# tobifinn/torch-assimilate

Hardware: AMD Instinct MI355X
Metric: local analyses/sec (LETKF, 40-member) (higher is better)
Workload: dtype f32

## Files before the change

torch-assimilate_amd/csrc/letkf_tile2_kernel.h:

```cpp
#pragma once
#include <type_traits>
#include "mia_common.h"
#include <hip/hip_ext.h>
#include "mia_kernels.h"
#include "mia_options.h"
#include "mia_tiles.h"
#ifdef MIA_TILE_STAMPS
namespace mia { constexpr int kT2StampN = 20, kT2StampTiles = 8192; static __device__ long long g_tile2_stamps[kT2StampTiles * kT2StampN]; }
#define MIA_TL_STAMP(i) do { if (lane == 0 && tile < mia::kT2StampTiles) mia::g_tile2_stamps[tile * mia::kT2StampN + 12 + (i)] = (long long)__builtin_amdgcn_s_memtime(); } while (0)
#endif
#include "mia_tile_localize.h"

namespace mia {

#ifdef MIA_TILE_STAMPS
#define T2_STAMP(i) do { if (lane == 0 && bid < kT2StampTiles) g_tile2_stamps[bid * kT2StampN + (i)] = (long long)__builtin_amdgcn_s_memtime(); } while (0)
#define T2_STAMP_HWID() do { if (lane == 0 && bid < kT2StampTiles) g_tile2_stamps[bid * kT2StampN + 9] = \
    (long long)(unsigned)__builtin_amdgcn_s_getreg((31 << 11) | 4) | ((long long)(unsigned)__builtin_amdgcn_s_getreg((31 << 11) | 20) << 32); } while (0)
#define T2_STAMP_REAL(i) do { if (lane == 0 && bid < kT2StampTiles) g_tile2_stamps[bid * kT2StampN + (i)] = (long long)__builtin_amdgcn_s_memrealtime(); } while (0)
#else
#define T2_STAMP(i) do { } while (0)
#define T2_STAMP_HWID() do { } while (0)
#define T2_STAMP_REAL(i) do { } while (0)
#endif

#ifndef MIA_TILE2_WAVES_UT2
#define MIA_TILE2_WAVES_UT2 4
#endif

template <int UT, int KT, bool MROWS, int LOC>
__device__ __forceinline__ void tile2_body(Tile2Params P, const Tile2Loc* loc, const int64_t bid) {
  constexpr int UMAX = 16 * UT, NB = (KT + 1) / 2, NKB = (UT + 1) / 2;
  extern __shared__ __attribute__((aligned(16))) unsigned char smem[];
  int lane = threadIdx.x, lr = lane & 15, h = lane >> 4;
  const int k = P.k, nc8 = P.nc8;
  const unsigned IMG = (unsigned)(UT * nc8) * 512u;
  unsigned char* zline = smem + IMG;
  int* ukey = reinterpret_cast<int*>(smem + IMG + 512);
  float* wdl = reinterpret_cast<float*>(ukey + UMAX);
  float* El = wdl + UMAX;

  const int64_t ntile = (P.ng + 15) >> 4;
  if (bid >= ntile) return;
  if (P.clr_counts) {
    const int ncl = *P.clr_n;
    for (int64_t i = bid * 64 + lane; i < ncl; i += ntile * 64) P.clr_counts[i] = 0;
    if (bid == 0 && lane == 0) {
      const unsigned e = *P.clr_err;
      if (e) { atomicOr(P.err_out, (int)(e << 3)); *P.clr_err = 0u; }
    }
  }
  const int64_t q8 = ntile >> 3, r8 = ntile & 7, xcd = bid & 7;
  const int64_t tile = (xcd < r8 ? xcd * (q8 + 1) : r8 * (q8 + 1) + (xcd - r8) * q8) + (bid >> 3);
  const int64_t p0 = tile << 4;
  const int npts = P.ng - p0 < 16 ? (int)(P.ng - p0) : 16;
  int64_t oc0 = P.o0 + p0;
  if (P.seg_len > 0) {
    const unsigned sgi = (unsigned)p0 / (unsigned)P.seg_len;
    oc0 = p0 - (int64_t)sgi * P.seg_len;
    P.Xa += (int64_t)sgi * P.seg_stride;
  }
  const unsigned ldxb = (unsigned)P.ldx * 4u, ldob = (unsigned)P.ldo * 4u;
  int lrc = lr < npts ? lr : npts - 1;
  bool colok = lr < npts;

#ifdef MIA_EXPERIMENTS
  const int prio_mode = (P.stagger >> 8) & 0xff, exp_trim = P.stagger >> 16;
  P.stagger &= 0xff;
  if (prio_mode == 1) __builtin_amdgcn_s_setprio(3);
  if (prio_mode >= 3) {
    const int wid = (int)(__builtin_amdgcn_s_getreg((4 << 11) | 4) & 0xf);
    const bool fast = prio_mode == 3 ? (wid & 1) : (prio_mode == 4 ? wid < 2 : (prio_mode == 5 ? wid == 0 : (wid % 3) == 0));
    if (fast) __builtin_amdgcn_s_setprio(3);
  }
  if (P.stagger > 0) {
    const int slot = (int)(__builtin_amdgcn_s_getreg((4 << 11) | 4) & 0xf);
    for (int i = 0; i < slot * P.stagger; ++i) __builtin_amdgcn_s_sleep(1);
  }
#endif
  T2_STAMP(0);
  T2_STAMP_HWID();
  T2_STAMP_REAL(10);
  int hdU = 0;
  int myidx[(UMAX + 63) / 64];
  f4w dreg[UT];
  if constexpr (LOC == 0) {
    const int4 hd = P.thdr[tile];
    hdU = hd.x;
#pragma unroll
    for (int r = 0; r < (UMAX + 63) / 64; ++r) {
      const int s = lane + 64 * r;
      myidx[r] = s < UMAX ? t2_ld<int32_t>(P.tidx + tile * UMAX, (unsigned)s * 4u) : -1;
    }
#pragma unroll
    for (int t = 0; t < UT; ++t) dreg[t] = t2_ld<f4w>(P.tD + (tile * UT + t) * 64, (unsigned)lane * 16u);
  } else {
    const TileLocOut lo = tile_localize<true, (LOC > 3 ? LOC - 4 : LOC), MIA_TAPER_GC, (LOC > 3)>(loc->scan, P.g0, P.ng, UT, tile, smem, lane);
    const TileLocLds LL(smem);
    hdU = lo.overflow ? -1 : lo.U;
    int mu[(UMAX + 63) / 64], du[UT][4];
#pragma unroll
    for (int r = 0; r < (UMAX + 63) / 64; ++r) {
      const int s = lane + 64 * r;
      mu[r] = LL.uinv[s < UMAX ? s : 0];
      mu[r] = (s < UMAX && !lo.overflow && mu[r] >= 0) ? mu[r] : kTlUmax;
    }
#pragma unroll
    for (int t = 0; t < UT; ++t)
#pragma unroll
      for (int qq = 0; qq < 4; ++qq) {
        du[t][qq] = LL.uinv[16 * t + 4 * h + qq];
        du[t][qq] = (!lo.overflow && du[t][qq] >= 0) ? du[t][qq] * 16 + lr : LL.zrow_off + lr;
      }
#pragma unroll
    for (int r = 0; r < (UMAX + 63) / 64; ++r) myidx[r] = LL.ukey[mu[r]];
#pragma unroll
    for (int t = 0; t < UT; ++t) {
      f4w v;
#pragma unroll
      for (int qq = 0; qq < 4; ++qq) v[qq] = LL.Wt[du[t][qq]];
      dreg[t] = v;
    }
    if (lane == 0) {
      if (lo.longest > loc->longest_bound) atomicMax(&loc->stats[0], lo.longest);
      else if ((tile & 63) == 0 && lo.longest > __hip_atomic_load(&loc->stats[0], __ATOMIC_RELAXED, __HIP_MEMORY_SCOPE_AGENT))
        atomicMax(&loc->stats[0], lo.longest);
      if (tile == 0) atomicOr(&loc->stats[3], kStepSampledLongest);
      if (lo.overflow) atomicAdd(&loc->stats[1], 1);
      if (lo.box_overflow) atomicOr(&loc->stats[1], MIA_TILE_BOX_OVERFLOW);
    }
    MIA_T2_SYNC();
  }
  int sg = 2 * (h & 1) + (h >> 1);
  auto load_xs = [&](int mi, float (&xr)[NB][8]) {
    const float* xbase = P.X + (int64_t)mi * k * P.ldx + P.g0 + p0;
#pragma unroll
    for (int b = 0; b < NB; ++b) {
      const int m0 = 8 * (4 * b + sg);
      if (b < NB - 1 || (k & 7) == 0) {
        const unsigned vo = (unsigned)(m0 < k ? m0 : 0) * ldxb + (unsigned)lrc * 4u;
#pragma unroll
        for (int i = 0; i < 8; ++i) xr[b][i] = t2_ld<float>(xbase, vo + (unsigned)i * ldxb);
      } else {
#pragma unroll
        for (int i = 0; i < 8; ++i) {
          const int mem = m0 + i;
          xr[b][i] = t2_ld<float>(xbase, (unsigned)(mem < k ? mem : k - 1) * ldxb + (unsigned)lrc * 4u);
        }
      }
    }
  };
  float xsb[NB][8];
  load_xs(0, xsb);
#pragma unroll
  for (int r = 0; r < (UMAX + 63) / 64; ++r) {
    const int s = lane + 64 * r;
    if (s < UMAX) ukey[s] = myidx[r];
  }
  for (int i = lane; i < 32; i += 64) reinterpret_cast<f4w*>(zline)[i] = f4w{0.f, 0.f, 0.f, 0.f};
  MIA_T2_SYNC();
  const int U = __builtin_amdgcn_readfirstlane(hdU);
  if (U < 0) {
    if (colok && h == 0) P.flags[p0 + lr] = MIA_FLAG_OVERFLOW;
    const float nanv = __builtin_nanf("");
    if (colok)
      for (int it = h; it < P.m * k; it += 4) P.Xa[(int64_t)it * P.ldo + oc0 + lr] = nanv;
    return;
  }
  T2_STAMP(1);
  {
    const int g = lane >> 4, hl = g & 1, gh = g >> 1;
    unsigned roff[UT][2];
#pragma unroll
    for (int t = 0; t < UT; ++t)
#pragma unroll
      for (int par = 0; par < 2; ++par) {
        const int idx = ukey[16 * t + ((lr - 8 * par) & 15)];
        roff[t][par] = (unsigned)(idx < 0 ? (int)P.zero_rec : idx) * (unsigned)P.rb + 16u * (unsigned)hl;
      }
    auto gather = [&](auto nc8c) {
      constexpr int NC8 = decltype(nc8c)::value;
      constexpr int NL = (UT * NC8 + 1) / 2;
#pragma unroll
      for (int u = 0; u < NL; ++u) {
        const int lA = 2 * u, lB = 2 * u + 1;
        const int tA = lA / NC8, cA = lA % NC8, tB = (lB / NC8) < UT ? lB / NC8 : UT - 1, cB = lB % NC8;
        const unsigned offA = roff[tA][cA & 1] + 32u * (unsigned)cA, offB = roff[tB][cB & 1] + 32u * (unsigned)cB;
        const unsigned off = gh ? offB : offA;
        const bool valid = 2 * u + gh < UT * NC8;
        if (valid)
          __builtin_amdgcn_global_load_lds(reinterpret_cast<const unsigned*>(P.rec + off),
                                           (__attribute__((address_space(3))) void*)(smem + u * 1024), 16, 0, 0);
      }
    };
    if (nc8 == 2 * KT - 1) gather(std::integral_constant<int, 2 * KT - 1>{});
    else gather(std::integral_constant<int, 2 * KT>{});
  }
  f2w tails[(UMAX + 63) / 64];
#pragma unroll
  for (int r = 0; r < (UMAX + 63) / 64; ++r) {
    const unsigned j = (unsigned)(myidx[r] < 0 ? (int)P.zero_rec : myidx[r]);
    tails[r] = *reinterpret_cast<const f2w*>(P.rec + (j * (unsigned)P.rb + 32u * (unsigned)nc8));
  }
  T2_STAMP(2);

  auto frag_off = [&](int t, int b) -> unsigned {
    const int c = 4 * b + sg;
    const unsigned col = (unsigned)((lr + 8 * (c & 1)) & 15) * 16u;
    return c < nc8 ? (unsigned)(t * nc8 + c) * 512u + col : IMG + col;
  };

  h8v GAh[UT][NKB], GAl[UT][NKB];
  float alpha = 0.0f;
  int deg = 0, tab_idx = 0, degmax = 0, pflag = 0;
  bool decl = false;
  auto split_x = [&](float (&xsb)[NB][8], float& xm, float& inv_sx, h8v (&xh)[NB], h8v (&xl)[NB]) {
      t2_split_x<NB, MROWS>(xsb, colok, sg, k, P.inv_k, xm, inv_sx, xh, xl);
    };
  float xm0, inv_sx0;
  f4w Z0[UT];
  {
    h8v xh[NB], xl[NB];
    split_x(xsb, xm0, inv_sx0, xh, xl);
#pragma unroll
    for (int t = 0; t < UT; ++t) Z0[t] = f4w{0.f, 0.f, 0.f, 0.f};
// ... 128 lines not shown
        const f4w d2 = dreg[t] * dreg[t];
        ad2[t] = alpha * d2;
        va[t] = Z[t] * d2;
#pragma unroll
        for (int q = 0; q < 4; ++q) zmaxf = __builtin_fmaxf(zmaxf, __builtin_fabsf(va[t][q]));
      }
      const unsigned zmax = t2_max_h(__float_as_uint(zmaxf));
      int es2;
      const float s2 = pow2_scale(zmax, 8, &es2);
      inv_s2 = __uint_as_float((unsigned)(127 - es2) << 23);
#pragma unroll
      for (int t = 0; t < UT; ++t) va[t] *= s2;
    }
    auto rhs_split = [&](const f4w (&tv)[UT], int kb, h8v& bh, h8v& bl) {
      float bv[8];
#pragma unroll
      for (int tt = 0; tt < 2; ++tt)
#pragma unroll
        for (int q = 0; q < 4; ++q) {
          const int tk = 2 * kb + tt < UT ? 2 * kb + tt : 0;
          bv[4 * tt + q] = 2 * kb + tt < UT ? tv[tk][q] : 0.0f;
        }
      split8(bv, bh, bl);
    };
    f4w y[UT];
    auto product = [&](const f4w (&tv)[UT]) {
      {
        h8v bh, bl;
        rhs_split(tv, 0, bh, bl);
#pragma unroll
        for (int t = 0; t < UT; ++t) y[t] = t2_mfma3(f4w{0.f, 0.f, 0.f, 0.f}, GAh[t][0], GAl[t][0], bh, bl);
      }
#pragma unroll
      for (int kb = 1; kb < NKB; ++kb)
        if (32 * kb < U) {
          h8v bh, bl;
          rhs_split(tv, kb, bh, bl);
#pragma unroll
          for (int t = 0; t < UT; ++t) y[t] = t2_mfma3(y[t], GAh[t][kb], GAl[t][kb], bh, bl);
        }
    };
    auto advance = [&](f4w (&vold)[UT], const f4w (&vcur)[UT], const float2 cj) {
      product(vcur);
#pragma unroll
      for (int t = 0; t < UT; ++t)
#pragma unroll
        for (int q = 0; q < 4; ++q) {
          const float tq = __builtin_fmaf(ad2[t][q], y[t][q], -vcur[t][q]);
          const float vn = __builtin_fmaf(2.0f, tq, -vold[t][q]);
          vold[t][q] = vn;
          aphi[t][q] = __builtin_fmaf(cj.x, vn, aphi[t][q]);
          apsi[t][q] = __builtin_fmaf(cj.y, vn, apsi[t][q]);
        }
    };
    product(va);
#pragma unroll
    for (int t = 0; t < UT; ++t)
#pragma unroll
      for (int q = 0; q < 4; ++q) {
        const float vq = __builtin_fmaf(ad2[t][q], y[t][q], -va[t][q]);
        vb[t][q] = vq;
        aphi[t][q] = __builtin_fmaf(c1.x, vq, c0.x * va[t][q]);
        apsi[t][q] = __builtin_fmaf(c1.y, vq, c0.y * va[t][q]);
      }
    int j = 2;
    for (; j + 1 <= degmax; j += 2) {
      const float2 cj = cn0, cj1 = cn1;
      cn0 = coef(j + 2); cn1 = coef(j + 3);
      advance(va, vb, cj);
      advance(vb, va, cj1);
    }
    if (j <= degmax) advance(va, vb, cn0);
    T2_STAMP(6);
    const float funs = inv_s2 * inv_sx;
    f4w xre[KT];
    {
      const float* xbase = P.X + (int64_t)mi * k * P.ldx + P.g0 + p0;
      const unsigned xo0 = (unsigned)(4 * h) * ldxb + (unsigned)lrc * 4u;
      const unsigned xolast = (unsigned)(k - 1) * ldxb + (unsigned)lrc * 4u;
#pragma unroll
      for (int tj = 0; tj < KT; ++tj)
#pragma unroll
        for (int q = 0; q < 4; ++q) {
          unsigned o = xo0 + (unsigned)(16 * tj + q) * ldxb;
          if (tj == KT - 1) o = o < xolast ? o : xolast;
          xre[tj][q] = t2_ld<float>(xbase, o);
        }
    }
    float zu = 0.0f;
#pragma unroll
    for (int t = 0; t < UT; ++t) {
      const f4w w4 = *reinterpret_cast<const f4w*>(wdl + 16 * t + 4 * h);
#pragma unroll
      for (int q = 0; q < 4; ++q) zu = fmaf(w4[q], apsi[t][q], zu);
    }
    zu = t2_add_h(zu) * (P.cs_psi * funs);
    const float mterm = xm + zu;
    h8v ph_[NKB], pl_[NKB];
#pragma unroll
    for (int kb = 0; kb < NKB; ++kb) rhs_split(aphi, kb, ph_[kb], pl_[kb]);
    const float fo = P.cs_phi * funs;
    const int tq = (lane & 15) >> 2, tp = lane & 3;
    f4w acc[KT];
    unsigned amax = 0u;
#pragma unroll
    for (int tj = 0; tj < KT; ++tj) {
      acc[tj] = f4w{0.f, 0.f, 0.f, 0.f};
      const int c = 2 * tj + (tp >> 1);
#pragma unroll
      for (int kb = 0; kb < NKB; ++kb)
        if (32 * kb < U) {
          s4v a4[2][2];
#pragma unroll
          for (int tt = 0; tt < 2; ++tt) {
            const int tb = 2 * kb + tt < UT ? 2 * kb + tt : 0;
            const unsigned col = (unsigned)((4 * h + tq + 8 * (c & 1)) & 15) * 16u + 8u * (unsigned)(tp & 1);
            const unsigned o = (c < nc8 && 2 * kb + tt < UT) ? (unsigned)(tb * nc8 + c) * 512u + col : IMG + col;
            a4[tt][0] = t2_tr_read(smem + o);
            a4[tt][1] = t2_tr_read(smem + o + 256);
          }
          typedef short s8v __attribute__((__vector_size__(8 * sizeof(short))));
          const s8v ahs = __builtin_shufflevector(a4[0][0], a4[1][0], 0, 1, 2, 3, 4, 5, 6, 7);
          const s8v als = __builtin_shufflevector(a4[0][1], a4[1][1], 0, 1, 2, 3, 4, 5, 6, 7);
          acc[tj] = t2_mfma3(acc[tj], __builtin_bit_cast(h8v, ahs), __builtin_bit_cast(h8v, als), ph_[kb], pl_[kb]);
        }
#pragma unroll
      for (int q = 0; q < 4; ++q) {
        acc[tj][q] = acc[tj][q] * fo + (mterm + P.f0 * (xre[tj][q] - xm));
        const unsigned ab = __float_as_uint(acc[tj][q]) & 0x7fffffffu;
        amax = ab > amax ? ab : amax;
      }
    }
    if (amax > 0x7149f2cau) pflag |= MIA_FLAG_NONFINITE;
    if (colok && !decl) {
      float* obase = P.Xa + (int64_t)mi * k * P.ldo + oc0;
      const unsigned olane = (unsigned)(4 * h) * ldob + (unsigned)lr * 4u;
#pragma unroll
      for (int tj = 0; tj < KT; ++tj)
#pragma unroll
        for (int q = 0; q < 4; ++q)
          if (tj < KT - 1 || 16 * tj + 4 * h + q < k)
            *reinterpret_cast<float*>(reinterpret_cast<char*>(obase) + (olane + (unsigned)(16 * tj + q) * ldob)) = acc[tj][q];
    } else {
      pflag = 0;
    }
  };
  row_tail(0, Z0, xm0, inv_sx0);
  if constexpr (MROWS) {
    for (int mi = 1; mi < P.m; ++mi) {
      asm volatile("" : "+v"(lane), "+v"(lr), "+v"(h));
      lrc = lr < npts ? lr : npts - 1;
      colok = lr < npts;
      sg = 2 * (h & 1) + (h >> 1);
      load_xs(mi, xsb);
      float xm, inv_sx;
      h8v xh[NB], xl[NB];
      split_x(xsb, xm, inv_sx, xh, xl);
      f4w Z[UT];
#pragma unroll
      for (int t = 0; t < UT; ++t) Z[t] = f4w{0.f, 0.f, 0.f, 0.f};
#pragma unroll
      for (int b = 0; b < NB; ++b) {
#pragma unroll
        for (int t = 0; t < UT; ++t) {
          const unsigned o = frag_off(t, b);
          const h8v ah = *reinterpret_cast<const h8v*>(smem + o), al = *reinterpret_cast<const h8v*>(smem + o + 256);
          Z[t] = t2_mfma3(Z[t], ah, al, xh[b], xl[b]);
        }
      }
      row_tail(mi, Z, xm, inv_sx);
    }
  }
  T2_STAMP(7);
  {
    const unsigned long long fb = __ballot(pflag != 0);
    const bool anyf = ((fb >> lr) & 0x0001000100010001ull) != 0ull;
    if (h == 0 && colok && !decl) P.flags[p0 + lr] = (anyf ? MIA_FLAG_NONFINITE : 0) | (deg << 8);
    if constexpr (LOC > 0) {
      if (fb != 0ull && lane == 0) atomicOr(&loc->stats[3], kStepNonfinite);
    }
  }
  T2_STAMP(8);
  T2_STAMP_REAL(11);
}


}
```

torch-assimilate_amd/csrc/letkf_tile2f.hip:

```cpp
#include "mia_common.h"
#include <hip/hip_ext.h>
#include "mia_kernels.h"
#include "mia_options.h"
#include "mia_tiles.h"
#include "mia_tile_launch.h"
#include "letkf_tile2_kernel.h"

namespace mia {

struct Tile2FParams { Tile2Params t; Tile2Loc loc; };

template <int UT, int KT, int NC, bool MROWS, int WAVES>
__global__ __launch_bounds__(64, WAVES)
void letkf_tile2f_kernel(Tile2FParams PF) { tile2_body<UT, KT, MROWS, NC>(PF.t, &PF.loc, (int64_t)blockIdx.y * gridDim.x + blockIdx.x); }

#ifdef MIA_TILE_STAMPS
extern "C" int mia_debug_tile2f_stamps(long long* host, int n_tiles) {
  if (n_tiles > kT2StampTiles) n_tiles = kT2StampTiles;
  return (int)hipMemcpyFromSymbol(host, HIP_SYMBOL(g_tile2_stamps), sizeof(long long) * kT2StampN * (size_t)n_tiles);
}
#endif

bool tile2f_covers(int m, int k, int ut, int n_coord) {
  const int kt = (k + 15) >> 4;
  return m >= 1 && ut >= 1 && ut <= 2 && kt >= 1 && kt <= 6 && n_coord >= 1 && n_coord <= MIA_MAX_COORD;
}

template <int UT, int KT, int NC, bool MROWS>
static int tile2f_launch_m(const Tile2FParams& pf, hipStream_t stream) {
  const size_t a = tile2_lds_bytes(UT, pf.t.k), b = tile_loc_lds(UT);
  const size_t lds = a > b ? a : b;
  constexpr int WAVES = MROWS ? 2 : MIA_TILE2_WAVES_UT2;
  return launch_blocks_carried(letkf_tile2f_kernel<UT, KT, NC, MROWS, WAVES>, (pf.t.ng + 15) >> 4, 64, lds, stream, [] {
    note_analysis_kernel("letkf_tile2f_kernel<%d, %d, %d, %s, %d>", UT, KT, NC, MROWS ? "true" : "false", WAVES);
  }, pf);
}

template <int UT, int KT, int NC>
static int tile2f_launch_n(const Tile2FParams& pf, hipStream_t stream) {
  return pf.t.m == 1 ? tile2f_launch_m<UT, KT, NC, false>(pf, stream) : tile2f_launch_m<UT, KT, NC, true>(pf, stream);
}

template <int UT>
static int tile2f_launch_u(const Tile2FParams& pf, int kt, hipStream_t stream) {
  return dispatch_upto<6>(kt, [&](auto kt_c) {
    return dispatch_among<7, 6, 5, 3, 2, 1>(pf.loc.scan.nc + (pf.loc.periodic ? 4 : 0), [&](auto nc) { return tile2f_launch_n<UT, kt_c(), nc()>(pf, stream); });
  });
}

int tile2f_launch(const Tile2Params& tp, const Tile2Loc& loc, int ut, int kt, hipStream_t stream) {
  if (!tile2f_covers(tp.m, tp.k, ut, loc.scan.nc) || !loc.stats) return MIA_ERR_UNSUPPORTED;
  Tile2FParams pf;
  pf.t = tp;
  pf.loc = loc;
#ifdef MIA_TILE2_SINGLE
  if (ut == 2 && kt == 3 && loc.scan.nc == 1) return tile2f_launch_n<2, 3, 1>(pf, stream);
  return MIA_ERR_UNSUPPORTED;
#else
  return ut == 1 ? tile2f_launch_u<1>(pf, kt, stream) : tile2f_launch_u<2>(pf, kt, stream);
#endif
}

}
```

torch-assimilate_amd/csrc/mia_tile_localize.h:

```cpp
#pragma once
#include "mia_common.h"
#include "mia_localize_dev.h"
#include "mia_tiles.h"

namespace mia {

#ifndef MIA_TL_STAMP
#define MIA_TL_STAMP(i) do { } while (0)
#endif
#define MIA_TL_SYNC() do { asm volatile("s_waitcnt lgkmcnt(0)" ::: "memory"); __builtin_amdgcn_wave_barrier(); } while (0)

__device__ __forceinline__ float gc_taper_fast(double d2, double four_c2, float inv_c, float c, float inv_c2) {
#pragma clang fp contract(off)
  const float d2f = (float)d2;
  const float r = __builtin_amdgcn_sqrtf(d2f) * inv_c;
  const float rinv = c * __builtin_amdgcn_rsqf(d2f);
  const float h1 = __builtin_fmaf(__builtin_fmaf(__builtin_fmaf(-0.25f, r, 0.5f), r, 0.625f), r, -5.0f / 3.0f);
  const float f1 = __builtin_fmaf(h1 * r, r, 1.0f);
  float t = (float)(four_c2 - d2) * inv_c2 * __builtin_amdgcn_rcpf(2.0f + r);
  t = __builtin_fmaxf(t, 0.0f);
  const float t2 = t * t;
  const float f2 = t2 * t2 * __builtin_fmaf(__builtin_fmaf(r, 1.0f / 12.0f, 1.0f / 6.0f), r, -1.0f / 24.0f) * rinv;
  return r < 1.0f ? f1 : f2;
}

__device__ __forceinline__ float gc_taper_fast_1d(double dx, double two_c, float inv_c, float c) {
#pragma clang fp contract(off)
  const float a = __builtin_fabsf((float)dx);
  const float r = a * inv_c;
  const float rinv = c * __builtin_amdgcn_rcpf(a);
  const float h1 = __builtin_fmaf(__builtin_fmaf(__builtin_fmaf(-0.25f, r, 0.5f), r, 0.625f), r, -5.0f / 3.0f);
  const float f1 = __builtin_fmaf(h1 * r, r, 1.0f);
  float t = (float)(two_c - __builtin_fabs(dx)) * inv_c;
  t = __builtin_fmaxf(t, 0.0f);
  const float t2 = t * t;
  const float f2 = t2 * t2 * __builtin_fmaf(__builtin_fmaf(r, 1.0f / 12.0f, 1.0f / 6.0f), r, -1.0f / 24.0f) * rinv;
  return r < 1.0f ? f1 : f2;
}

constexpr int kTlUmax = 96;
constexpr int kTlMaxRows = 64;

struct TileLocLds {
  double* gxs;
  int* cgs;
  int* ukey;
  int* uinv;
  double* cox;
  int* coj;
  float* Wt;
  static constexpr int zrow_off = -16;
  __device__ __forceinline__ explicit TileLocLds(unsigned char* base) {
    gxs = reinterpret_cast<double*>(base);
    cox = gxs + 16 * MIA_MAX_COORD;
    cgs = reinterpret_cast<int*>(cox + 64 * MIA_MAX_COORD);
    ukey = cgs + 16 * MIA_MAX_COORD;
    uinv = ukey + kTlUmax + 16;
    coj = uinv + kTlUmax;
    Wt = reinterpret_cast<float*>(coj + 64) + 16;
  }
};
static inline size_t tile_loc_lds(int ut) {
  return (16 + 64) * MIA_MAX_COORD * sizeof(double) + 16 * MIA_MAX_COORD * sizeof(int) + (2 * kTlUmax + 16 + 64) * sizeof(int) +
         (size_t)16 * (ut * 16 + 1) * sizeof(float);
}

struct TileLocOut {
  int U;
  int longest;
  int npts;
  bool overflow;
  bool box_overflow;
};

template <bool BUCKET, int NC, int TAPER, bool PERIODIC = false>
__device__ __forceinline__ TileLocOut tile_localize(const ScanParams& q, int64_t g0, int64_t ng, int ut, int64_t tile,
                                                    unsigned char* tl_lds, int lane) {
  const TileLocLds lds_(tl_lds);
  double* gxs = lds_.gxs; int* cgs = lds_.cgs; int* ukey = lds_.ukey; int* uinv = lds_.uinv; float* Wt = lds_.Wt;
  double* cox = lds_.cox; int* coj = lds_.coj;
  const int cl = lane & 15, pg = lane >> 4;
  const int UMAX = 16 * ut;
  const IndexHeader* hd = q.hdr;
  constexpr int nc = NC;
  const int64_t p0 = tile << 4;
  const int npts = ng - p0 < 16 ? (int)(ng - p0) : 16;
  MIA_TL_STAMP(0);
  if (lane < 16) {
    const int64_t pt = g0 + p0 + (lane < npts ? lane : npts - 1);
    for (int c = 0; c < MIA_MAX_COORD; ++c) {
      double gx = 0.0;
      int cg = 0;
      if (c < nc) {
        gx = q.grid[pt * nc + c];
        if constexpr (PERIODIC) point_cell(hd, c, gx, &gx, &cg);
        else cg = cell_coord(gx, hd->mn[c], hd->invh[c], hd->n[c]);
      }
      gxs[lane * MIA_MAX_COORD + c] = gx;
      cgs[lane * MIA_MAX_COORD + c] = cg;
    }
  }
  for (int s = lane; s < kTlUmax; s += 64) uinv[s] = -1;
  if (lane < 16) { Wt[TileLocLds::zrow_off + lane] = 0.0f; ukey[kTlUmax + lane] = -1; }
  MIA_TL_SYNC();
  MIA_TL_STAMP(1);
  int lo[MIA_MAX_COORD], hi[MIA_MAX_COORD];
  double perL[NC], perI[NC];
  bool pairwise = false;
  if constexpr (PERIODIC) {
#pragma unroll
    for (int c = 0; c < NC; ++c) { perL[c] = hd->period[c]; perI[c] = hd->inv_period[c]; }
  }
  for (int c = 0; c < MIA_MAX_COORD; ++c) {
    int mn = cgs[cl * MIA_MAX_COORD + c], mx = mn;
    bool cyc = false;
    int cg0 = 0, ncyc = 1;
    if constexpr (PERIODIC) {
      if (c < nc && hd->period[c] > 0.0) {
        cyc = true;
        ncyc = hd->n[c];
        cg0 = __builtin_amdgcn_readfirstlane(cgs[c]);
        int rel = mn - cg0;
        rel = rel < 0 ? rel + ncyc : rel;
        rel = rel > ncyc / 2 ? rel - ncyc : rel;
        const bool odd = mn < 0 || cg0 < 0 || cg0 + rel < 0 || cg0 + rel >= ncyc;
        pairwise = pairwise || __ballot(odd) != 0ull;
        mn = mx = rel;
      }
    }
#define MIA_TL_ROW_STEP(ctrl) do { const int a_ = __builtin_amdgcn_update_dpp(0, mn, ctrl, 0xf, 0xf, false), b_ = __builtin_amdgcn_update_dpp(0, mx, ctrl, 0xf, 0xf, false); \
                                   mn = a_ < mn ? a_ : mn; mx = b_ > mx ? b_ : mx; } while (0)
    MIA_TL_ROW_STEP(0xB1); MIA_TL_ROW_STEP(0x4E); MIA_TL_ROW_STEP(0x124); MIA_TL_ROW_STEP(0x128);
#undef MIA_TL_ROW_STEP
    lo[c] = mn - 1 < 0 ? 0 : mn - 1;
    hi[c] = mx + 1 > hd->n[c] - 1 ? hd->n[c] - 1 : mx + 1;
    if constexpr (PERIODIC) {
      if (cyc) {
        lo[c] = cg0 + mn - 1;
        hi[c] = cg0 + mx + 1;
        if (ncyc < 3 || hi[c] - lo[c] + 1 > ncyc || cg0 < 0) { lo[c] = 0; hi[c] = ncyc - 1; pairwise = true; }
      }
    }
    if (c >= nc) { lo[c] = 0; hi[c] = 0; }
    lo[c] = __builtin_amdgcn_readfirstlane(lo[c]);
    hi[c] = __builtin_amdgcn_readfirstlane(hi[c]);
  }
  const int last = nc - 1;
  bool empty = false;
  for (int c = 0; c < nc; ++c) empty = empty || lo[c] > hi[c];
  const int n0 = nc >= 2 ? hi[0] - lo[0] + 1 : 1;
  const int n1 = nc == 3 ? hi[1] - lo[1] + 1 : 1;
  const long long nrows = empty ? 0 : (long long)n0 * n1;
  bool overflow = nrows > kTlMaxRows;
  bool box_overflow = overflow;
  int ubase = 0;
  double gxr[4][NC];
#pragma unroll
  for (int i = 0; i < 4; ++i)
#pragma unroll
    for (int c = 0; c < NC; ++c) gxr[i][c] = gxs[(4 * pg + i) * MIA_MAX_COORD + c];
  int grp[NC];
#pragma unroll
  for (int c = 0; c < NC; ++c) grp[c] = NC == 1 ? 0 : q.group[c];
  const int n_r = NC == 1 ? 1 : q.n_r;
  const float epsf = q.eps_f;
  double fc2[MIA_MAX_RADII];
  float icf[MIA_MAX_RADII], ccf[MIA_MAX_RADII], ic2f[MIA_MAX_RADII];
#pragma unroll
  for (int r = 0; r < MIA_MAX_RADII; ++r) { fc2[r] = q.four_c2[r]; icf[r] = q.inv_c_f[r]; ccf[r] = q.c_f[r]; ic2f[r] = q.inv_c2_f[r]; }
  const double twoc0 = 2.0 * q.cc[0];
  struct Cand { int oj; double ox[NC]; };
  auto fetch = [&](int64_t pos) {
    Cand cd;
    cd.oj = q.sorted[pos];
#pragma unroll
    for (int c = 0; c < NC; ++c) cd.ox[c] = q.sxyz[pos * NC + c];
    return cd;
  };
  bool ptok[4];
#pragma unroll
  for (int i = 0; i < 4; ++i) ptok[i] = 4 * pg + i < npts;
  int cntl[4] = {0, 0, 0, 0};
  auto disp = [&](double ox, int i, int c) -> double {
    if constexpr (PERIODIC) {
      if (pairwise) return cyc_disp(ox, gxr[i][c], 0.0, perL[c] > 0.0, perL[c], perI[c]);
    }
// ... 258 lines not shown
```

torch-assimilate_amd/csrc/mia_tiles.h:

```cpp
#pragma once
#include "mia_common.h"

namespace mia {

constexpr int kTileSlack = 8;

static inline int tile_ut_for(int p_max) {
  const int ut = (p_max + kTileSlack + 15) >> 4;
  return ut < 1 ? 1 : ut;
}

struct TileListLayout { size_t hdr, idx, D, bytes; int ut; int64_t ntile; };
static inline TileListLayout tile_list_layout(int64_t ng, int ut) {
  TileListLayout L;
  L.ut = ut;
  L.ntile = (ng + 15) >> 4;
  size_t o = 0;
  L.hdr = o; o = align_up(o + (size_t)(L.ntile > 0 ? L.ntile : 1) * 16, 256);
  L.idx = o; o = align_up(o + (size_t)(L.ntile > 0 ? L.ntile : 1) * 16 * ut * sizeof(int32_t), 256);
  L.D = o; o = align_up(o + (size_t)(L.ntile > 0 ? L.ntile : 1) * ut * 1024, 256);
  L.bytes = o;
  return L;
}

// ... 106 lines not shown
  u2v r = __builtin_amdgcn_permlane32_swap(u, u, false, false);
  u = r.x > r.y ? r.x : r.y;
  r = __builtin_amdgcn_permlane16_swap(u, u, false, false);
  return r.x > r.y ? r.x : r.y;
}
template <int NB, bool TIED>
__device__ __forceinline__ void t2_split_x(float (&xsb)[NB][8], const bool colok, const int sg, const int k, const float inv_k,
                                           float& xm, float& inv_sx, h8v (&xh)[NB], h8v (&xl)[NB]) {
#pragma clang fp contract(off)
  float xs = 0.0f;
  unsigned xmax = 0u;
  if ((k & 7) == 0) {
    float lm[NB];
#pragma unroll
    for (int b = 0; b < NB; ++b) lm[b] = (colok && 8 * (4 * b + sg) < k) ? 1.0f : 0.0f;
#pragma unroll
    for (int b = 0; b < NB; ++b)
#pragma unroll
      for (int i = 0; i < 8; ++i) xs = __builtin_fmaf(xsb[b][i], lm[b], xs);
    xm = t2_add_h(xs) * inv_k;
    float xmaxf = 0.0f;
#pragma unroll
    for (int b = 0; b < NB; ++b) {
      const float xml = xm * lm[b];
#pragma unroll
      for (int i = 0; i < 8; ++i) {
        xsb[b][i] = __builtin_fmaf(xsb[b][i], lm[b], -xml);
        xmaxf = __builtin_fmaxf(xmaxf, __builtin_fabsf(xsb[b][i]));
      }
    }
    xmax = __float_as_uint(xmaxf);
  } else {
#pragma unroll
    for (int b = 0; b < NB; ++b)
#pragma unroll
      for (int i = 0; i < 8; ++i) {
        const bool live = colok && 8 * (4 * b + sg) + i < k;
        xsb[b][i] = live ? xsb[b][i] : 0.0f;
        xs += xsb[b][i];
      }
    xm = t2_add_h(xs) * inv_k;
#pragma unroll
    for (int b = 0; b < NB; ++b)
#pragma unroll
      for (int i = 0; i < 8; ++i) {
        const bool live = colok && 8 * (4 * b + sg) + i < k;
        xsb[b][i] = live ? xsb[b][i] - xm : 0.0f;
        const unsigned a = __float_as_uint(xsb[b][i]) & 0x7fffffffu;
        xmax = a > xmax ? a : xmax;
      }
  }
  xmax = t2_max_h(xmax);
  int esx;
  const float sx = pow2_scale(xmax, 9, &esx);
  inv_sx = __uint_as_float((unsigned)(127 - esx) << 23);
#pragma unroll
  for (int b = 0; b < NB; ++b) {
    float t8[8];
#pragma unroll
    for (int i = 0; i < 8; ++i) t8[i] = xsb[b][i] * sx;
    if constexpr (TIED) split8_tied(t8, xh[b], xl[b]);
    else split8(t8, xh[b], xl[b]);
  }
}
__device__ __forceinline__ unsigned t2_wave_max_u32(unsigned u) {
  unsigned t;
  t = (unsigned)__builtin_amdgcn_update_dpp(0, (int)u, 0xB1, 0xf, 0xf, false); u = u > t ? u : t;
  t = (unsigned)__builtin_amdgcn_update_dpp(0, (int)u, 0x4E, 0xf, 0xf, false); u = u > t ? u : t;
  t = (unsigned)__builtin_amdgcn_update_dpp(0, (int)u, 0x124, 0xf, 0xf, false); u = u > t ? u : t;
  t = (unsigned)__builtin_amdgcn_update_dpp(0, (int)u, 0x128, 0xf, 0xf, false); u = u > t ? u : t;
  const unsigned a = (unsigned)__builtin_amdgcn_readlane((int)u, 0), b = (unsigned)__builtin_amdgcn_readlane((int)u, 16);
  const unsigned c = (unsigned)__builtin_amdgcn_readlane((int)u, 32), d = (unsigned)__builtin_amdgcn_readlane((int)u, 48);
  const unsigned ab = a > b ? a : b, cd = c > d ? c : d;
  return ab > cd ? ab : cd;
}
__device__ __forceinline__ f4w t2_mfma3(f4w acc, const h8v ah, const h8v al, const h8v bh, const h8v bl) {
  acc = __builtin_amdgcn_mfma_f32_16x16x32_f16(al, bh, acc, 0, 0, 0);
  acc = __builtin_amdgcn_mfma_f32_16x16x32_f16(ah, bl, acc, 0, 0, 0);
  return __builtin_amdgcn_mfma_f32_16x16x32_f16(ah, bh, acc, 0, 0, 0);
}
template <typename T>
__device__ __forceinline__ T t2_ld(const void* base, unsigned byte_off) {
  return *reinterpret_cast<const T*>(reinterpret_cast<const char*>(base) + byte_off);
}
typedef short s4v __attribute__((__vector_size__(4 * sizeof(short))));
__device__ __forceinline__ s4v t2_tr_read(const unsigned char* lds_addr) {
  return __builtin_amdgcn_ds_read_tr16_b64_v4i16((__attribute__((address_space(3))) s4v*)lds_addr);
}


struct SplitPackJob { const float* Yb; const float* d; unsigned char* rec; int k; };

__device__ inline void pack_split_wave(const SplitPackJob& J, int64_t P, int64_t block, float* lds) {
  const int lane = threadIdx.x & 63;
  const int k = J.k, nc8 = (k + 7) >> 3, rb = 32 * nc8 + 16;
  const int ls = (k + 1) | 1;
  float* scl = lds + 64 * ls;
  const int64_t j0 = block * 64;
  const int64_t j = j0 + lane;
  const bool real = j < P;
  const int64_t jc = real ? j : (P > 0 ? P - 1 : 0);
  const float dj = (real && P > 0) ? J.d[jc] : 0.0f;
  constexpr int kRowsInFlight = 40;
  for (int i0 = 0; i0 < k; i0 += kRowsInFlight) {
    float v[kRowsInFlight];
#pragma unroll
    for (int u = 0; u < kRowsInFlight; ++u) {
      const int i = i0 + u < k ? i0 + u : k - 1;
      v[u] = (P > 0) ? J.Yb[(int64_t)i * P + jc] : 0.0f;
    }
#pragma unroll
    for (int u = 0; u < kRowsInFlight; ++u)
      if (i0 + u < k) lds[lane * ls + i0 + u] = real ? v[u] : 0.0f;
  }
  do { asm volatile("s_waitcnt lgkmcnt(0)" ::: "memory"); __builtin_amdgcn_wave_barrier(); } while (0);
  unsigned mx = 0u;
  for (int i = 0; i < k; ++i) {
    const unsigned a = __float_as_uint(lds[lane * ls + i]) & 0x7fffffffu;
    mx = a > mx ? a : mx;
  }
  int es;
  const float sc = pow2_scale(mx, 9, &es);
  const float wd = dj * sc;
  const bool bad = mx >= 0x7f800000u || !(fabsf(wd) < 3.0e38f);
  scl[lane] = sc;
  if (j <= P) {
    const float E = bad ? __builtin_nanf("") : __uint_as_float((unsigned)(127 - es) << 23);
    *reinterpret_cast<f4w*>(J.rec + j * rb + 32 * nc8) = f4w{wd, E, 0.0f, 0.0f};
  }
  do { asm volatile("s_waitcnt lgkmcnt(0)" ::: "memory"); __builtin_amdgcn_wave_barrier(); } while (0);
  const int nvalid = P + 1 - j0 < 64 ? (int)(P + 1 - j0) : 64;
  const int nq = nvalid * nc8;
  int r = lane / nc8, c = lane - r * nc8;
  const int dr = 64 / nc8, dc = 64 - dr * nc8;
  for (int q = lane; q < nq; q += 64) {
    const float s = scl[r];
    float x[8];
#pragma unroll
    for (int i = 0; i < 8; ++i) x[i] = 8 * c + i < k ? lds[r * ls + 8 * c + i] * s : 0.0f;
    h8v hi, lo;
    split8(x, hi, lo);
    unsigned char* o = J.rec + (j0 + r) * rb + 32 * c;
    *reinterpret_cast<h8v*>(o) = hi;
    *reinterpret_cast<h8v*>(o + 16) = lo;
    r += dr; c += dc;
    if (c >= nc8) { c -= nc8; ++r; }
  }
}

static inline size_t split_pack_lds(int k) { return ((size_t)64 * ((k + 1) | 1) + 64) * sizeof(float); }

__device__ __forceinline__ void pack_split_lean_request(const SplitPackJob& J, int64_t P, int64_t block, float* lds) {
  const int lane = threadIdx.x & 63;
  const int64_t j = block * 64 + lane;
  const int64_t jc = j < P ? j : (P > 0 ? P - 1 : 0);
  if (P > 0)
    for (int i = 0; i < J.k; ++i)
      __builtin_amdgcn_global_load_lds(reinterpret_cast<const unsigned*>(J.Yb + (int64_t)i * P + jc),
                                       (__attribute__((address_space(3))) void*)(lds + i * 64), 4, 0, 0);
}
__device__ __forceinline__ void pack_split_lean_finish(const SplitPackJob& J, int64_t P, int64_t block, const float* lds) {
  const int lane = threadIdx.x & 63;
  const int k = J.k, nc8 = (k + 7) >> 3, rb = 32 * nc8 + 16;
  const int64_t j = block * 64 + lane;
  const bool real = j < P;
  const float dj = (real && P > 0) ? J.d[j] : 0.0f;
// ... 68 lines not shown
```

Measured before the change: 2.558 billion.

## Cut register pressure by re-reading kernel args and using scalar-base row addressing

Moves the parameter-derived setup to after tile localization and re-reads the kernel argument struct through an opaque offset, so the Params copy need not stay live in registers across the localize phase. Replaces per-lane 64-bit address arithmetic for X loads and output stores with scalar (SGPR) per-row base pointers plus a lane offset. Removes the overflow and negative-slot clamps on the uinv lookups by moving the ukey sentinel slots in front of the table so that index -1 lands on them. This depends on the LDS layout change being correct for the overflow case and adds SGPR pressure, in exchange for fewer VGPRs and VALU address ops.

```diff
diff --git a/torch-assimilate_amd/csrc/letkf_tile2_kernel.h b/torch-assimilate_amd/csrc/letkf_tile2_kernel.h
--- a/torch-assimilate_amd/csrc/letkf_tile2_kernel.h
+++ b/torch-assimilate_amd/csrc/letkf_tile2_kernel.h
@@ -29,16 +29,10 @@
 #endif
 
 template <int UT, int KT, bool MROWS, int LOC>
-__device__ __forceinline__ void tile2_body(Tile2Params P, const Tile2Loc* loc, const int64_t bid) {
+__device__ __forceinline__ void tile2_body(Tile2Params P, const Tile2Loc* loc, const int64_t bid, const Tile2Params* pk = nullptr) {
   constexpr int UMAX = 16 * UT, NB = (KT + 1) / 2, NKB = (UT + 1) / 2;
   extern __shared__ __attribute__((aligned(16))) unsigned char smem[];
   int lane = threadIdx.x, lr = lane & 15, h = lane >> 4;
-  const int k = P.k, nc8 = P.nc8;
-  const unsigned IMG = (unsigned)(UT * nc8) * 512u;
-  unsigned char* zline = smem + IMG;
-  int* ukey = reinterpret_cast<int*>(smem + IMG + 512);
-  float* wdl = reinterpret_cast<float*>(ukey + UMAX);
-  float* El = wdl + UMAX;
 
   const int64_t ntile = (P.ng + 15) >> 4;
   if (bid >= ntile) return;
@@ -53,16 +47,6 @@
   const int64_t q8 = ntile >> 3, r8 = ntile & 7, xcd = bid & 7;
   const int64_t tile = (xcd < r8 ? xcd * (q8 + 1) : r8 * (q8 + 1) + (xcd - r8) * q8) + (bid >> 3);
   const int64_t p0 = tile << 4;
-  const int npts = P.ng - p0 < 16 ? (int)(P.ng - p0) : 16;
-  int64_t oc0 = P.o0 + p0;
-  if (P.seg_len > 0) {
-    const unsigned sgi = (unsigned)p0 / (unsigned)P.seg_len;
-    oc0 = p0 - (int64_t)sgi * P.seg_len;
-    P.Xa += (int64_t)sgi * P.seg_stride;
-  }
-  const unsigned ldxb = (unsigned)P.ldx * 4u, ldob = (unsigned)P.ldo * 4u;
-  int lrc = lr < npts ? lr : npts - 1;
-  bool colok = lr < npts;
 
 #ifdef MIA_EXPERIMENTS
   const int prio_mode = (P.stagger >> 8) & 0xff, exp_trim = P.stagger >> 16;
@@ -96,22 +80,18 @@
     for (int t = 0; t < UT; ++t) dreg[t] = t2_ld<f4w>(P.tD + (tile * UT + t) * 64, (unsigned)lane * 16u);
   } else {
     const TileLocOut lo = tile_localize<true, (LOC > 3 ? LOC - 4 : LOC), MIA_TAPER_GC, (LOC > 3)>(loc->scan, P.g0, P.ng, UT, tile, smem, lane);
+    P = *t2_args_again(pk);
+    loc = t2_args_again(loc);
     const TileLocLds LL(smem);
     hdU = lo.overflow ? -1 : lo.U;
+    static_assert(64 * ((UMAX + 63) / 64) <= kTlUmax, "every lane's slot must lie inside the slot table");
     int mu[(UMAX + 63) / 64], du[UT][4];
 #pragma unroll
-    for (int r = 0; r < (UMAX + 63) / 64; ++r) {
-      const int s = lane + 64 * r;
-      mu[r] = LL.uinv[s < UMAX ? s : 0];
-      mu[r] = (s < UMAX && !lo.overflow && mu[r] >= 0) ? mu[r] : kTlUmax;
-    }
+    for (int r = 0; r < (UMAX + 63) / 64; ++r) mu[r] = LL.uinv[lane + 64 * r];
 #pragma unroll
     for (int t = 0; t < UT; ++t)
 #pragma unroll
-      for (int qq = 0; qq < 4; ++qq) {
-        du[t][qq] = LL.uinv[16 * t + 4 * h + qq];
-        du[t][qq] = (!lo.overflow && du[t][qq] >= 0) ? du[t][qq] * 16 + lr : LL.zrow_off + lr;
-      }
+      for (int qq = 0; qq < 4; ++qq) du[t][qq] = LL.uinv[16 * t + 4 * h + qq] * 16 + lr;
 #pragma unroll
     for (int r = 0; r < (UMAX + 63) / 64; ++r) myidx[r] = LL.ukey[mu[r]];
 #pragma unroll
@@ -131,16 +111,35 @@
     }
     MIA_T2_SYNC();
   }
+  const int k = P.k, nc8 = P.nc8;
+  const unsigned IMG = (unsigned)(UT * nc8) * 512u;
+  unsigned char* zline = smem + IMG;
+  int* ukey = reinterpret_cast<int*>(smem + IMG + 512);
+  float* wdl = reinterpret_cast<float*>(ukey + UMAX);
+  float* El = wdl + UMAX;
+  const int npts = P.ng - p0 < 16 ? (int)(P.ng - p0) : 16;
+  int64_t oc0 = P.o0 + p0;
+  if (P.seg_len > 0) {
+    const unsigned sgi = (unsigned)p0 / (unsigned)P.seg_len;
+    oc0 = p0 - (int64_t)sgi * P.seg_len;
+    P.Xa += (int64_t)sgi * P.seg_stride;
+  }
+  const unsigned ldxb = (unsigned)P.ldx * 4u, ldob = (unsigned)P.ldo * 4u;
+  int lrc = lr < npts ? lr : npts - 1;
+  bool colok = lr < npts;
   int sg = 2 * (h & 1) + (h >> 1);
   auto load_xs = [&](int mi, float (&xr)[NB][8]) {
     const float* xbase = P.X + (int64_t)mi * k * P.ldx + P.g0 + p0;
+    t2_gptr xrow[8];
+#pragma unroll
+    for (int i = 0; i < 8; ++i) xrow[i] = MROWS ? t2_gptr() : t2_sbase(xbase + i * P.ldx);
 #pragma unroll
     for (int b = 0; b < NB; ++b) {
       const int m0 = 8 * (4 * b + sg);
       if (b < NB - 1 || (k & 7) == 0) {
         const unsigned vo = (unsigned)(m0 < k ? m0 : 0) * ldxb + (unsigned)lrc * 4u;
 #pragma unroll
-        for (int i = 0; i < 8; ++i) xr[b][i] = t2_ld<float>(xbase, vo + (unsigned)i * ldxb);
+        for (int i = 0; i < 8; ++i) xr[b][i] = MROWS ? t2_ld<float>(xbase, vo + (unsigned)i * ldxb) : t2_ld_s<float>(xrow[i], vo);
       } else {
 #pragma unroll
         for (int i = 0; i < 8; ++i) {
@@ -435,9 +434,12 @@
       for (int tj = 0; tj < KT; ++tj)
 #pragma unroll
         for (int q = 0; q < 4; ++q) {
-          unsigned o = xo0 + (unsigned)(16 * tj + q) * ldxb;
-          if (tj == KT - 1) o = o < xolast ? o : xolast;
-          xre[tj][q] = t2_ld<float>(xbase, o);
+          if (!MROWS && tj < KT - 1) {
+            xre[tj][q] = t2_ld_s<float>(t2_sbase(xbase + (16 * tj + q) * P.ldx), xo0);
+          } else {
+            const unsigned o = xo0 + (unsigned)(16 * tj + q) * ldxb;
+            xre[tj][q] = t2_ld<float>(xbase, o < xolast ? o : xolast);
+          }
         }
     }
     float zu = 0.0f;
@@ -492,8 +494,10 @@
       for (int tj = 0; tj < KT; ++tj)
 #pragma unroll
         for (int q = 0; q < 4; ++q)
-          if (tj < KT - 1 || 16 * tj + 4 * h + q < k)
-            *reinterpret_cast<float*>(reinterpret_cast<char*>(obase) + (olane + (unsigned)(16 * tj + q) * ldob)) = acc[tj][q];
+          if (tj < KT - 1 || 16 * tj + 4 * h + q < k) {
+            if constexpr (MROWS) *reinterpret_cast<float*>(reinterpret_cast<char*>(obase) + (olane + (unsigned)(16 * tj + q) * ldob)) = acc[tj][q];
+            else t2_st_s<float>(t2_sbase(obase + (16 * tj + q) * P.ldo), olane, acc[tj][q]);
+          }
     } else {
       pflag = 0;
     }
diff --git a/torch-assimilate_amd/csrc/letkf_tile2f.hip b/torch-assimilate_amd/csrc/letkf_tile2f.hip
--- a/torch-assimilate_amd/csrc/letkf_tile2f.hip
+++ b/torch-assimilate_amd/csrc/letkf_tile2f.hip
@@ -12,7 +12,7 @@
 
 template <int UT, int KT, int NC, bool MROWS, int WAVES>
 __global__ __launch_bounds__(64, WAVES)
-void letkf_tile2f_kernel(Tile2FParams PF) { tile2_body<UT, KT, MROWS, NC>(PF.t, &PF.loc, (int64_t)blockIdx.y * gridDim.x + blockIdx.x); }
+void letkf_tile2f_kernel(Tile2FParams PF) { tile2_body<UT, KT, MROWS, NC>(PF.t, &PF.loc, (int64_t)blockIdx.y * gridDim.x + blockIdx.x, &PF.t); }
 
 #ifdef MIA_TILE_STAMPS
 extern "C" int mia_debug_tile2f_stamps(long long* host, int n_tiles) {
diff --git a/torch-assimilate_amd/csrc/mia_tile_localize.h b/torch-assimilate_amd/csrc/mia_tile_localize.h
--- a/torch-assimilate_amd/csrc/mia_tile_localize.h
+++ b/torch-assimilate_amd/csrc/mia_tile_localize.h
@@ -54,8 +54,8 @@
     gxs = reinterpret_cast<double*>(base);
     cox = gxs + 16 * MIA_MAX_COORD;
     cgs = reinterpret_cast<int*>(cox + 64 * MIA_MAX_COORD);
-    ukey = cgs + 16 * MIA_MAX_COORD;
-    uinv = ukey + kTlUmax + 16;
+    ukey = cgs + 16 * MIA_MAX_COORD + 16;
+    uinv = ukey + kTlUmax;
     coj = uinv + kTlUmax;
     Wt = reinterpret_cast<float*>(coj + 64) + 16;
   }
@@ -101,7 +101,7 @@
     }
   }
   for (int s = lane; s < kTlUmax; s += 64) uinv[s] = -1;
-  if (lane < 16) { Wt[TileLocLds::zrow_off + lane] = 0.0f; ukey[kTlUmax + lane] = -1; }
+  if (lane < 16) { Wt[TileLocLds::zrow_off + lane] = 0.0f; ukey[lane - 16] = -1; }
   MIA_TL_SYNC();
   MIA_TL_STAMP(1);
   int lo[MIA_MAX_COORD], hi[MIA_MAX_COORD];
diff --git a/torch-assimilate_amd/csrc/mia_tiles.h b/torch-assimilate_amd/csrc/mia_tiles.h
--- a/torch-assimilate_amd/csrc/mia_tiles.h
+++ b/torch-assimilate_amd/csrc/mia_tiles.h
@@ -212,6 +212,26 @@
 template <typename T>
 __device__ __forceinline__ T t2_ld(const void* base, unsigned byte_off) {
   return *reinterpret_cast<const T*>(reinterpret_cast<const char*>(base) + byte_off);
+}
+template <typename T>
+__device__ __forceinline__ const T* t2_args_again(const T* p) {
+  unsigned z = 0u;
+  asm volatile("" : "+s"(z));
+  return reinterpret_cast<const T*>(reinterpret_cast<const char*>(p) + z);
+}
+typedef __attribute__((address_space(1))) char* t2_gptr;
+__device__ __forceinline__ t2_gptr t2_sbase(const void* p) {
+  t2_gptr g = (t2_gptr)const_cast<void*>(p);
+  asm("" : "+s"(g));
+  return g;
+}
+template <typename T>
+__device__ __forceinline__ T t2_ld_s(t2_gptr sbase, unsigned byte_off) {
+  return *reinterpret_cast<const __attribute__((address_space(1))) T*>(sbase + byte_off);
+}
+template <typename T>
+__device__ __forceinline__ void t2_st_s(t2_gptr sbase, unsigned byte_off, T v) {
+  *reinterpret_cast<__attribute__((address_space(1))) T*>(sbase + byte_off) = v;
 }
 typedef short s4v __attribute__((__vector_size__(4 * sizeof(short))));
 __device__ __forceinline__ s4v t2_tr_read(const unsigned char* lds_addr) {
```

After: 2.583 billion (median of 6 runs). Within noise of the previous version (+1.0%).
